# BindsNET/bindsnet

Hardware: AMD Instinct MI355X
Metric: simulated timesteps/sec (whole node), DiehlAndCook2015 784->400 batch32 (higher is better)
Workload: dtype f32

## Files before the change

### bindsnet_amd/csrc/snn_dc2015_async.hip

```cpp
#include <limits.h>
#include <stdlib.h>
#include "snn_dc2015.hpp"
#include "snn_dc2015_tile.hpp"

namespace {

constexpr int ACW = 4;
constexpr int ANT = 512;
constexpr int kCrossRing = 4;
constexpr int kWinRing = 8;
constexpr int kWinGr = 11;
constexpr int kArbRing = 32;
constexpr unsigned kAPoll = 400000u;
constexpr unsigned kAbortPay = 0xFFFFFFFEu;

__device__ __forceinline__ uint32_t win_tag(int e) { return (uint32_t)(e + 1) & 1023u; }

__device__ __forceinline__ void report(int *status, int code) {
    if (status) atomicCAS(status, 0, code);
}

__device__ __forceinline__ const DcCtx &cold(const DcCtx &) {
    const __attribute__((address_space(4))) DcCtx *p = (const __attribute__((address_space(4))) DcCtx *)__builtin_amdgcn_kernarg_segment_ptr();
    asm volatile("" : "+s"(p));
// ... 92 lines not shown
        cb = blk;
    };
#pragma unroll
    for (int u = 0; u < 8; ++u) if (u < nL) add(ix[u], wx[u] * 1.0f, wy[u] * 1.0f);
    for (int u = 8; u < nL; ++u) {
        const int ii2 = (int)lx[st + u];
        add(ii2, ws[ii2 * CW + pq] * 1.0f, DUAL ? ws2[ii2 * CW + pq] * 1.0f : 0.f);
    }
    const int GL = (Nin >> 4) >> 4;
    auto combine = [&](float G) __attribute__((always_inline)) -> float {
        const float G1 = __shfl_down(G, 1, 4), G2 = __shfl_down(G, 2, 4), G3 = __shfl_down(G, 3, 4);
        const float Gs[4] = {G, G1, G2, G3};
        float A2 = 0.0f;
#pragma unroll
        for (int k = 0; k < 4; ++k) if (k < GL) A2 = A2 + Gs[k];
        float Gl = 0.0f;
#pragma unroll
        for (int k = 0; k < 4; ++k) if (k == GL) Gl = Gs[k];
        const float res = ((0.0f + Gl) + A2) + 0.0f;
        return 0.0f + res;
    };
    if (DUAL) out2 = combine(c1_ + c0_);
    return combine(a1 + a0);
}

template <int K>
__device__ __forceinline__ float quad_down(float v) {
    constexpr int ctrl = K == 1 ? 0x39 : (K == 2 ? 0x0E : 0x03);
    return __int_as_float(__builtin_amdgcn_mov_dpp(__float_as_int(v), ctrl, 0xF, 0xF, true));
}

__device__ __forceinline__ float4 x_current_f4(const float *ws, const uint32_t *dg, int B, int Nin, int pb, int pL, bool tailcol) {
    constexpr uint32_t GM = (1u << GCB) - 1u;
    const uint16_t *lstX = (const uint16_t *)dg;
    const uint32_t *rowmask = dg + B * (LX / 2) + 40;
    const uint16_t *arows = (const uint16_t *)(rowmask + Nin);
    const uint16_t *lst2 = arows + 4 * ((Nin + 1) / 2);
    const uint32_t *gcnt = (const uint32_t *)(lst2 + B * LX);
    const uint32_t *gqn = gcnt + B;
    float r[4];
    if (tailcol) {
        const uint32_t gc = gcnt[pb];
        const int st = (pL > 0 ? (int)(gc & GM) : 0) + (pL > 1 ? (int)((gc >> GCB) & GM) : 0) + (pL > 2 ? (int)((gc >> (2 * GCB)) & GM) : 0);
        const int nL = (int)((gc >> (GCB * pL)) & GM);
        const uint16_t *l2 = lst2 + pb * LX;
        const int n4 = Nin >> 2, nfull = n4 >> 4;
        int ix[8]; float4 wx[8];
#pragma unroll
        for (int u = 0; u < 8; ++u) ix[u] = min((int)l2[min(st + u, LX - 1)], Nin - 1);
#pragma unroll
        for (int u = 0; u < 8; ++u) wx[u] = *(const float4 *)(ws + ix[u] * 4);
        float a0[4] = {0.f, 0.f, 0.f, 0.f}, a1[4] = {0.f, 0.f, 0.f, 0.f}, a2[4] = {0.f, 0.f, 0.f, 0.f};
        int cb = -1;
        auto add = [&](int pos, const float4 &w) __attribute__((always_inline)) {
            int blk = pos >> 4;
            blk = blk < nfull ? blk : nfull;
            const bool nb = blk != cb, ng = (blk >> 4) != (cb >> 4);
            const float t[4] = {w.x * 1.0f, w.y * 1.0f, w.z * 1.0f, w.w * 1.0f};
#pragma unroll
            for (int q = 0; q < 4; ++q) {
                const float s1 = a1[q] + a0[q];
                a1[q] = nb ? s1 : a1[q];
                a0[q] = nb ? 0.f : a0[q];
                const float s2 = a2[q] + a1[q];
                a2[q] = ng ? s2 : a2[q];
                a1[q] = ng ? 0.f : a1[q];
                a0[q] += t[q];
            }
            cb = blk;
        };
#pragma unroll
        for (int u = 0; u < 8; ++u) if (u < nL) add(ix[u] >> 2, wx[u]);
        for (int u = 8; u < nL; ++u) {
            const int i = (int)l2[st + u];
            add(i >> 2, *(const float4 *)(ws + i * 4));
        }
        const bool closeb = cb != nfull, closeg = closeb && (nfull >> 4) != (cb >> 4);
        float v[4];
#pragma unroll
        for (int q = 0; q < 4; ++q) {
            float b0 = a0[q], b1 = a1[q], b2 = a2[q];
            if (closeb) { b1 += b0; b0 = 0.f; if (closeg) { b2 += b1; b1 = 0.f; } }
            v[q] = ((b0 + b1) + b2) + 0.0f;
        }
        if (pL == 0) {
            const int s4 = (int)(gc & GM) + (int)((gc >> GCB) & GM) + (int)((gc >> (2 * GCB)) & GM) + (int)((gc >> (3 * GCB)) & GM);
            const int n5 = (int)((gc >> (4 * GCB)) & GM);
            for (int u = 0; u < n5; ++u) {
                const int i = (int)l2[s4 + u];
                const float4 w = *(const float4 *)(ws + i * 4);
                v[0] += w.x * 1.0f; v[1] += w.y * 1.0f; v[2] += w.z * 1.0f; v[3] += w.w * 1.0f;
            }
        }
#pragma unroll
        for (int q = 0; q < 4; ++q) {
            const float v1 = __shfl_down(v[q], 1, 4), v2 = __shfl_down(v[q], 2, 4), v3 = __shfl_down(v[q], 3, 4);
            r[q] = 0.0f + (((v[q] + v1) + v2) + v3);
        }
        return make_float4(r[0], r[1], r[2], r[3]);
    }
    const uint32_t gq = gqn[pb];
    const int st = (pL > 0 ? (int)(gq & GM) : 0) + (pL > 1 ? (int)((gq >> GCB) & GM) : 0) + (pL > 2 ? (int)((gq >> (2 * GCB)) & GM) : 0);
    const int nL = (int)((gq >> (GCB * pL)) & GM);
    const uint16_t *lx = lstX + pb * LX;
    int ix[8]; float4 wx[8];
    const int last = st + max(nL, 1) - 1;
#pragma unroll
    for (int u = 0; u < 8; ++u) ix[u] = (int)lx[min(st + u, last)];
#pragma unroll
    for (int u = 0; u < 8; ++u) wx[u] = *(const float4 *)(ws + ix[u] * 4);
    float a0[4] = {0.f, 0.f, 0.f, 0.f}, a1[4] = {0.f, 0.f, 0.f, 0.f};
    int cb = -1;
    const int nfull = Nin >> 4;
    auto add = [&](int pos, const float4 &w, float live) __attribute__((always_inline)) {
        int blk = pos >> 4;
        blk = blk < nfull ? blk : nfull;
        const float same = blk == cb ? 1.f : 0.f, diff = 1.f - same;
        const float t[4] = {w.x * live, w.y * live, w.z * live, w.w * live};
#pragma unroll
        for (int q = 0; q < 4; ++q) {
            a1[q] = __builtin_fmaf(a0[q], diff, a1[q]);
            a0[q] = __builtin_fmaf(a0[q], same, t[q]);
        }
        cb = blk;
    };
#pragma unroll
    for (int u = 0; u < 8; ++u) add(ix[u], wx[u], u < nL ? 1.0f : 0.0f);
    for (int u = 8; u < nL; ++u) {
        const int i2 = (int)lx[st + u];
        add(i2, *(const float4 *)(ws + i2 * 4), 1.0f);
    }
    const int GL = (Nin >> 4) >> 4;
#pragma unroll
    for (int q = 0; q < 4; ++q) {
        const float G = a1[q] + a0[q];
        const float G1 = quad_down<1>(G), G2 = quad_down<2>(G), G3 = quad_down<3>(G);
        const float Gs[4] = {G, G1, G2, G3};
        float A2 = 0.0f;
#pragma unroll
        for (int k = 0; k < 4; ++k) if (k < GL) A2 = A2 + Gs[k];
        float Gl = 0.0f;
#pragma unroll
        for (int k = 0; k < 4; ++k) if (k == GL) Gl = Gs[k];
        const float res = ((0.0f + Gl) + A2) + 0.0f;
        r[q] = 0.0f + res;
    }
    return make_float4(r[0], r[1], r[2], r[3]);
}

__device__ __forceinline__ void scan_entry(const DcCtx &c, int *w0, int *cnt0, int tid) {
    const int B = c.B, N = c.N;
    if (tid < 2 * MAXB) { w0[tid] = -1; cnt0[tid] = 0; }
    __syncthreads();
    for (int k = tid; k < B * N; k += ANT) {
        if (c.sE[k]) { const int b = k / N; atomicAdd(&cnt0[b], 1); w0[b] = k - b * N; }
        if (c.sI[k]) { const int b = k / N; atomicAdd(&cnt0[MAXB + b], 1); w0[MAXB + b] = k - b * N; }
    }
    __syncthreads();
}

constexpr int kWinPollSleep = 1;
struct WinPre { unsigned long long g0; bool have; };
__device__ __forceinline__ WinPre win_prefetch(const DcCtx &c, int e, int myb) {
    WinPre p; p.g0 = granule_load(c.wing + (size_t)(e & (kWinRing - 1)) * kWinGr + myb / 3); p.have = true;
    return p;
}
__device__ __forceinline__ int sample_winner(const DcCtx &c, const int *w0, int e, int myb, bool &bad, WinPre pre = WinPre{0ull, false}) {
    if (e < 0) return w0[(e == -1 ? 0 : MAXB) + myb];
    const unsigned long long *gr = c.wing + (size_t)(e & (kWinRing - 1)) * kWinGr + myb / 3;
    const uint32_t tag = win_tag(e);
    unsigned long long x0 = pre.have ? pre.g0 : granule_load(gr);
    for (unsigned spins = 0; __any((uint32_t)(x0 >> 54) != tag); ++spins) {
        if (spins > kAPoll) { bad = true; report(cold(c).status, SNN_ERR_TIMEOUT); return -1; }
        __builtin_amdgcn_s_sleep(kWinPollSleep);
        x0 = granule_load(gr);
    }
    if (__any((int)((x0 >> 48) & 63u) == 63)) { bad = true; return -1; }
    const uint32_t w = (uint32_t)(x0 >> (16 * (myb % 3))) & 0xFFFFu;
    return w == 0xFFFFu ? -1 : (int)(w & 0x7FFu);
}

#define AMARKW(k, th) do { if constexpr (TIMING) { if (c.dbg && g == c.dbg_wg && tid == (th)) c.dbg[(size_t)t * 24 + (k)] = (long long)wall_clock64(); } } while (0)
#define AMARK(k) do { if constexpr (TIMING) { if (wave == 0 && c.dbg_wg >= 0) mk[k] = (long long)wall_clock64(); } } while (0)
#define AMARK2(k) do { if constexpr (TIMING) { if (wave == 2 && c.dbg_wg >= 0) mk[k] = (long long)wall_clock64(); } } while (0)
#define AMARK2_FLUSH() do { if constexpr (TIMING) { if (c.dbg && g == c.dbg_wg && tid == 128 && t >= 1) { _Pragma("unroll") for (int k_ = 19; k_ < 24; ++k_) c.dbg[(size_t)(t - 1) * 24 + k_] = mk[k_]; } } } while (0)
#define AMARK_FLUSH() do { if constexpr (TIMING) { if (c.dbg && g == c.dbg_wg && tid == 0) { _Pragma("unroll") for (int k_ = 0; k_ < 19; ++k_) { \
        const bool early_ = k_ == 0 || k_ == 9 || k_ == 10 || k_ == 7 || k_ == 11 || k_ == 18; \
        if (k_ != 3 && k_ != 17 && (early_ || t >= 1)) c.dbg[(size_t)(early_ ? t : t - 1) * 24 + k_] = mk[k_]; } } } } while (0)

__device__ __forceinline__ float vgpr(float x) { float r; asm volatile("v_mov_b32 %0, %1" : "=v"(r) : "s"(x)); return r; }
__device__ __forceinline__ snn_lif_params vgpr_params(snn_lif_params p) {
    p.decay = vgpr(p.decay); p.rest = vgpr(p.rest); p.reset = vgpr(p.reset); p.thresh = vgpr(p.thresh); p.refrac = vgpr(p.refrac);
    p.dt = vgpr(p.dt); p.lbound = vgpr(p.lbound); p.trace_decay = vgpr(p.trace_decay); p.trace_scale = vgpr(p.trace_scale);
    return p;
}
struct PPar { float nu0, nu1, dt, wmin, wmax; int use_dt, has_min, has_max; };

__device__ __forceinline__ float4 postpre_row_nowin(const PPar &c, float4 w4, uint32_t m, const float *xnu0) {
    float w[4] = {w4.x, w4.y, w4.z, w4.w};
    if (c.nu0 != 0.f) {
        float a0[4] = {0.f, 0.f, 0.f, 0.f}, a1[4] = {0.f, 0.f, 0.f, 0.f};
        int cblk = 0;
        while (m) {
            const int b = __ffs(m) - 1; m &= m - 1;
            const float4 xn = *(const float4 *)(xnu0 + b * 4);
            const float xv[4] = {xn.x, xn.y, xn.z, xn.w};
            const float same = (b >> 4) == cblk ? 1.f : 0.f, diff = 1.f - same;
            cblk = b >> 4;
#pragma unroll
            for (int q = 0; q < 4; ++q) {
                a1[q] = __builtin_fmaf(a0[q], diff, a1[q]);
                a0[q] = __builtin_fmaf(a0[q], same, 1.0f * xv[q]);
            }
        }
#pragma unroll
        for (int q = 0; q < 4; ++q) {
            float uu = ((a0[q] + a1[q]) + 0.f) + 0.0f;
            if (c.use_dt) uu = uu * c.dt;
            w[q] = w[q] - uu;
        }
    }
    if (c.nu1 != 0.f) {
#pragma unroll
        for (int q = 0; q < 4; ++q) {
            float uu = 0.f;
            if (c.use_dt) uu = uu * c.dt;
            w[q] = w[q] + uu;
        }
    }
#pragma unroll
    for (int q = 0; q < 4; ++q) {
        if (c.has_min && w[q] < c.wmin) w[q] = c.wmin;
        if (c.has_max && w[q] > c.wmax) w[q] = c.wmax;
    }
    return make_float4(w[0], w[1], w[2], w[3]);
}

__device__ __forceinline__ float postpre_elem(const PPar &c, int B, int Nin, const float *xnu0, float w, int i, int q, uint32_t m, uint32_t cm,
                                              int bst, float xw, const float *xs, bool have_x, float xval) {
    constexpr int CW = ACW;
    if (c.nu0 != 0.f) {
        float uu = 0.f;
        if (m) {
            CascadeT acc; acc.init(false);
            while (m) {
                const int b = __ffs(m) - 1; m &= m - 1;
                acc.add(b, 1.0f * (b == bst ? xw : xnu0[b * CW + q]), B);
            }
            uu = acc.finish(B);
        }
        if (c.use_dt) uu = uu * c.dt;
        w = w - uu;
    }
    if (c.nu1 != 0.f) {
        float uu = 0.f;
        if (cm) {
            CascadeT acc; acc.init(false);
            while (cm) {
                const int b = __ffs(cm) - 1; cm &= cm - 1;
                acc.add(b, (have_x ? xval : xs[b * Nin + i]) * (1.0f * c.nu1), B);
            }
            uu = acc.finish(B);
        }
        if (c.use_dt) uu = uu * c.dt;
        w = w + uu;
    }
    if (c.has_min && w < c.wmin) w = c.wmin;
    if (c.has_max && w > c.wmax) w = c.wmax;
    return w;
}

constexpr int kXChunk = 256;
__device__ __forceinline__ int x_chunks(const DcCtx &c) { return c.x_traces ? (c.B * c.Nin + kXChunk - 1) / kXChunk : 0; }

__device__ __forceinline__ void async_producer(const DcCtx &c, unsigned char *smem, int p) {
    const int T = c.T, tid = threadIdx.x;
    for (int e = p; e <= T; e += c.NP) {
        const int flags = dc_prep_entry<ANT>(c, smem, e, c.dig + (size_t)e * c.DW);
        if (tid == 0) {
            if (flags & 5) atomicOr(c.tbad, 1);
            __hip_atomic_store(&c.dready[e], (flags & 5) ? 2 : 1, __ATOMIC_RELEASE, __HIP_MEMORY_SCOPE_AGENT);
            __hip_atomic_fetch_add(&c.dready[T + 1], 1, __ATOMIC_RELEASE, __HIP_MEMORY_SCOPE_AGENT);
        }
    }
    const int n = c.B * c.Nin, nch = x_chunks(c);
    for (int ch = p; ch < nch; ch += c.NP) {
        const int k = ch * kXChunk + tid;
        if (tid < kXChunk && k < n) { if (c.x_additive) xtrace_body<true>(c, n, k); else xtrace_body<false>(c, n, k); }
        __syncthreads();
        if (tid == 0) __hip_atomic_fetch_add(&c.dready[T + 2], 1, __ATOMIC_RELEASE, __HIP_MEMORY_SCOPE_AGENT);
    }
    if (c.rasX) {
        const size_t n16 = ((size_t)T * c.B * c.Nin) >> 4;
        const uint4 *src = (const uint4 *)c.in;
        uint4 *dst = (uint4 *)c.rasX;
        for (size_t k = (size_t)p * ANT + tid; k < n16; k += (size_t)c.NP * ANT) dst[k] = src[k];
    }
}

__device__ __forceinline__ int need_entry(const DcCtx &c, int e, bool &all) {
    const int T = c.T;
    int r;
    if (__hip_atomic_load(&c.dready[T + 1], __ATOMIC_RELAXED, __HIP_MEMORY_SCOPE_AGENT) == T + 1) {
        all = true;
        r = 0;
    } else {
        for (unsigned spins = 0;; ++spins) {
            r = __hip_atomic_load(&c.dready[e], __ATOMIC_RELAXED, __HIP_MEMORY_SCOPE_AGENT);
            if (r) break;
            if (spins > kAPoll) return -1;
            __builtin_amdgcn_s_sleep(4);
        }
    }
    __builtin_amdgcn_fence(__ATOMIC_ACQUIRE, "agent");
    if (all) r = __hip_atomic_load(c.tbad, __ATOMIC_RELAXED, __HIP_MEMORY_SCOPE_AGENT) != 0 ? 2 : 1;
    return r;
}
__device__ __forceinline__ int need_xtr(const DcCtx &c, bool &all) {
    const int nch = x_chunks(c);
    for (unsigned spins = 0;; ++spins) {
        if (__hip_atomic_load(&c.dready[c.T + 2], __ATOMIC_RELAXED, __HIP_MEMORY_SCOPE_AGENT) == nch) break;
        if (spins > kAPoll) return -1;
        __builtin_amdgcn_s_sleep(4);
    }
    __builtin_amdgcn_fence(__ATOMIC_ACQUIRE, "agent");
    all = true;
    return 1;
}

template <bool TIMING, bool FT>
__device__ __forceinline__ void async_compute(const DcCtx &c, unsigned char *smem) {
    constexpr int CW = ACW, TT = AT, NT = ANT, NTW = TT / 64, SPW = 64 / CW, SPG = 16 / CW, NBC = NT - TT, TI0 = NT - TT;
    const int B = FT ? MAXB : c.B, Nin = c.Nin, N = c.N, T = c.T;
    int *ctl = (int *)(smem + OC_CTL);
    float *xnu0 = (float *)(smem + OC_XNU0);
    float *xnu0s = (float *)(smem + OC_XNU0S);
    float *curX = (float *)(smem + OC_CURX);
    float *curXwin = (float *)(smem + OC_CURXW);
    int *spfin = (int *)(smem + OC_SPFIN);
    int *thc = (int *)(smem + OC_THC);
    uint32_t *colmask = (uint32_t *)(smem + OC_COLM);
    uint32_t *colx = (uint32_t *)(smem + OC_COLX);
    uint32_t *colres = (uint32_t *)(smem + OC_COLRES);
    float *xwinv = (float *)(smem + OC_XWINV);
    int *xcnt = (int *)(smem + OC_XCNT);
    int *w0 = (int *)(smem + OC_W0), *cnt0 = (int *)(smem + OC_C0);
    float *wtile = (float *)(smem + OC_WT);
    float *wieT = wtile + (size_t)Nin * CW;
    float *weiT = wieT + (size_t)N * CW;
    const int DGS = (c.DGW + 63) & ~63;
    uint32_t *dgbuf = (uint32_t *)(weiT + (size_t)N * CW);
    float *wbak = (float *)(dgbuf + 2 * DGS);
    float *wwin = wbak + (size_t)Nin * CW;

    const int tid = threadIdx.x, lane = tid & 63, wave = tid >> 6;
    const int g = (int)blockIdx.x, c0 = g * CW;
    const bool is_ai = tid >= TI0;
    const int ptile = is_ai ? tid - TI0 : tid;
    const int jj = ptile % CW, bl = ptile / CW, j = c0 + jj;
    const bool colv = FT ? true : j < N, tailcol = c0 >= (N / 32) * 32;
    const bool mine = FT ? tid < TT : (tid < TT && bl < B && colv);
    const bool mine_i = FT ? is_ai : (is_ai && bl < B && colv);
    const unsigned kst = (unsigned)(bl * N + j);
    const int NGS = c.G * NTW;
    const snn_lif_params pE = vgpr_params(c.pE.lif), pI = vgpr_params(c.pI);
    const float theta_plus = vgpr(c.pE.theta_plus), theta_decay = vgpr(c.pE.theta_decay);
    const PPar pp = {vgpr(c.nu0), vgpr(c.nu1), vgpr(c.dt), vgpr(c.wmin), vgpr(c.wmax), c.use_dt, c.has_min, c.has_max};
    const bool e_learning = c.pE.learning != 0;

    if (tid < 32) ctl[tid] = 0;
    if (tid < 2 * CW) { thc[tid] = 0; colx[tid] = 0; colmask[tid] = 0; colres[tid & 3] = 0; xwinv[tid & 3] = 0.f; }
    scan_entry(c, w0, cnt0, tid);
    bool offdiag = false, multi0 = false;
    for (int k = tid; k < Nin * CW; k += NT) {
        const int i = k / CW, q = k % CW;
        wtile[k] = (c0 + q < N) ? c.Wxe[i * N + c0 + q] : 0.f;
        wbak[k] = 0.f; wwin[k] = 0.f;
    }
    for (int k = tid; k < N * CW; k += NT) {
        const int i = k / CW, q = k % CW;
        wieT[k] = (c0 + q < N) ? c.Wie[i * N + c0 + q] : 0.f;
        const float we = (c0 + q < N) ? c.Wei[i * N + c0 + q] : 0.f;
        weiT[k] = we;
        offdiag = offdiag || (i != c0 + q && we != 0.f);
    }
    if (tid < 2 * MAXB) multi0 = cnt0[tid] > 1;
    if (offdiag || multi0) ctl[0] = 1;
    const int nchunk = c.DGW >> 2;
    uint4 dg0 = make_uint4(0, 0, 0, 0), dg1 = dg0, dg2 = dg0;
#define DIGEST_LOAD(e) do { const uint4 *src_ = (const uint4 *)(c.dig + (size_t)(e) * c.DW); dg0 = src_[min(tid, nchunk - 1)]; \
                            dg1 = src_[min(tid + NT, nchunk - 1)]; dg2 = src_[min(tid + 2 * NT, nchunk - 1)]; } while (0)
#define DIGEST_STORE(e) do { uint4 *dst_ = (uint4 *)(dgbuf + ((e) & 1) * DGS); if (tid < nchunk) dst_[tid] = dg0; \
                             if (tid + NT < nchunk) dst_[tid + NT] = dg1; if (tid + 2 * NT < nchunk) dst_[tid + 2 * NT] = dg2; } while (0)
    int pend = 0;
    int dig01 = 1;
    if (c.NP != 0) {
        bool dig_all = false;
        const int r0 = need_entry(c, 0, dig_all), r1 = (T >= 1 && !dig_all) ? need_entry(c, 1, dig_all) : 1;
        dig01 = r0 != 1 ? r0 : r1;
        if (dig01 != 1) { ctl[0] = 1; if (tid == 0) report(c.status, dig01 < 0 ? SNN_ERR_TIMEOUT : SNN_ERR_RETRY); }
        const int p0 = (dig_all ? 0 : 1) | (c.x_traces ? 2 : 0);
        asm volatile("v_mov_b32 %0, %1" : "=v"(pend) : "s"(p0));
    }
#define PENDING(bit) (__builtin_amdgcn_readfirstlane(pend) & (bit))
    if (dig01 >= 0) DIGEST_LOAD(0);
    DIGEST_STORE(0);
    if (T >= 1) { if (dig01 >= 0) DIGEST_LOAD(1); DIGEST_STORE(1); }
    uint4 dg3 = make_uint4(0, 0, 0, 0);
#define DIGEST_LOAD_E(e) do { const uint4 *src_ = (const uint4 *)(c.dig + (size_t)(e) * c.DW); const int d_ = tid - TT; dg0 = src_[min(d_, nchunk - 1)]; \
                              dg1 = src_[min(d_ + NBC, nchunk - 1)]; dg2 = src_[min(d_ + 2 * NBC, nchunk - 1)]; dg3 = src_[min(d_ + 3 * NBC, nchunk - 1)]; } while (0)
#define DIGEST_STORE_E(e) do { uint4 *dst_ = (uint4 *)(dgbuf + ((e) & 1) * DGS); const int d_ = tid - TT; if (d_ < nchunk) dst_[d_] = dg0; \
                               if (d_ + NBC < nchunk) dst_[d_ + NBC] = dg1; if (d_ + 2 * NBC < nchunk) dst_[d_ + 2 * NBC] = dg2; \
                               if (d_ + 3 * NBC < nchunk) dst_[d_ + 3 * NBC] = dg3; } while (0)
    float r_v = 0.f, r_r = 0.f, r_th = 0.f, x_cur = 0.f, x_before = 0.f;
    bool last_s = false;
    if (mine) {
        r_v = c.vE[kst]; r_r = c.rE[kst]; r_th = c.theta[j];
        x_cur = pE.traces ? c.xE[kst] : 0.f;
        last_s = c.sE[kst] != 0;
    }
    if (mine_i) {
        r_v = c.vI[kst]; r_r = c.rI[kst];
        x_cur = pI.traces ? c.xI[kst] : 0.f;
        last_s = c.sI[kst] != 0;
    }
    if (tid < TT) {
        float xn = 0.f;
        if (bl < B && colv && pE.traces) xn = trace_next(x_cur, 0, pE.trace_decay, pE.trace_scale, pE.traces_additive);
        xnu0[tid] = xn * pp.nu0; xnu0[TT + tid] = 0.f; xnu0s[tid] = 0.f;
        curX[tid] = 0.f; curX[TT + tid] = 0.f; curXwin[tid] = 0.f;
        spfin[tid] = (mine && last_s) ? 1 : 0;
    }
    asm volatile("s_waitcnt vmcnt(0)" ::: "memory");
    __syncthreads();
    bool bad = ctl[0] != 0;
    if (bad && tid == 0) report(c.status, SNN_ERR_RETRY);
    for (int qt = tid; qt < B * CW * 4; qt += NT) {
        const int pb = qt / (CW * 4), pq = (qt >> 2) % CW, pL = qt & 3;
        float unused = 0.f;
        const float v = x_current4<false>(wtile, wtile, unused, dgbuf, B, Nin, pb, pq, pL, tailcol);
        if (pL == 0 && c0 + pq < N) curX[pb * CW + pq] = v;
    }
    lds_barrier();
    bool sp_prev = false;
    bool crossed_prev = false;
    unsigned long long prevE = 0ull;
    int published = 0;
    WinPre pre_w = WinPre{0ull, false};
    const bool learn_pp = c.learning && c.rule == SNN_RULE_POSTPRE;

    if constexpr (TIMING) {
        if (c.dbg && tid == 0) {
            c.dbg[(size_t)24 * (T + 1) + ((size_t)T * 256 + g) * 4 + 2] = (long long)(__builtin_amdgcn_s_getreg((31 << 11) | 20) & 0xF);
            c.dbg[(size_t)24 * (T + 1) + ((size_t)T * 256 + g) * 4 + 3] = (long long)(__builtin_amdgcn_s_getreg((31 << 11) | 4) & 0xFFFFFF);
        }
    }
    long long mk[24] = {0, 0, 0, 0, 0, 0, 0, 0, 0, 0, 0, 0, 0, 0, 0, 0, 0, 0, 0, 0, 0, 0, 0, 0};
    (void)mk;
    bool prev_anyx = true;
    auto step_loop = [&](auto role_c) __attribute__((always_inline)) {
    constexpr int ROLE = decltype(role_c)::value;
    constexpr bool R_TILE = ROLE == 0, R_F4 = ROLE == 1, R_W4 = ROLE == 2, R_AI = ROLE == 3, R_NT = ROLE != 0;
    (void)R_W4; (void)R_AI; (void)R_F4;
    for (int t = 0; t <= T; ++t) {
        const bool phaseB = t < T;
        const int par = t & 1;
        const uint32_t *dgn = dgbuf + (par ^ 1) * DGS;
        const int *meta = (const int *)(dgn + B * (LX / 2));
        const uint32_t *rowmask = dgn + B * (LX / 2) + 40;
        const uint16_t *arows = (const uint16_t *)(rowmask + Nin);
        const bool do_stdp = phaseB && learn_pp;
        const bool full = t == 0;
        AMARK(0);
        AMARK2_FLUSH();
        if constexpr (TIMING) { if (c.dbg && tid == 0 && c.dbg_wg >= 0) c.dbg[(size_t)24 * (T + 1) + ((size_t)t * 256 + g) * 4 + 0] = (long long)wall_clock64(); }
        if (t + 2 <= T && R_NT) {
            if (PENDING(1)) {
                bool all = false;
                const int r = need_entry(cold(c), t + 2, all);
                if (r != 1) { ctl[0] = 1; report(cold(c).status, r < 0 ? SNN_ERR_TIMEOUT : SNN_ERR_RETRY); }
                if (all) pend &= ~1;
            }
            DIGEST_LOAD_E(t + 2);
        }
        float cx_plain = 0.f;
        int thc_prev = 0;
        if (R_TILE) { cx_plain = curX[par * TT + tid]; thc_prev = thc[(par ^ 1) * CW + jj]; }
        if (ctl[0]) { bad = true; break; }
        AMARK(9);
        uint32_t wonm = 0;
        if (learn_pp && prev_anyx) {
#pragma unroll
            for (int q = 0; q < CW; ++q) wonm |= (__builtin_amdgcn_readfirstlane((int)colmask[par * CW + q]) != 0 ? 1u : 0u) << q;
        }
        AMARK(10);
        if (!phaseB) {
            if (wonm)
                for (int i = tid; i < Nin; i += NT) {
                    float4 v = *(const float4 *)(wtile + i * 4);
                    const float4 ww = *(const float4 *)(wwin + i * 4);
                    if (wonm & 1u) v.x = ww.x;
                    if (wonm & 2u) v.y = ww.y;
                    if (wonm & 4u) v.z = ww.z;
                    if (wonm & 8u) v.w = ww.w;
                    *(float4 *)(wtile + i * 4) = v;
                }
            break;
        }
        if (R_TILE) {
// ... 162 lines not shown
                }
                lds_barrier();
#pragma unroll
                for (int q = 0; q < CW; ++q) if (__popc(xq[q]) > 1) cmq[q] = (uint32_t)__builtin_amdgcn_readfirstlane((int)colres[q]);
                if (R_TILE) {
                    float v = xn0[tid];
                    const uint32_t xj = jj == 0 ? xq[0] : (jj == 1 ? xq[1] : (jj == 2 ? xq[2] : xq[3]));
                    const uint32_t cj = jj == 0 ? cmq[0] : (jj == 1 ? cmq[1] : (jj == 2 ? cmq[2] : cmq[3]));
                    if (bl < B && colv && __popc(xj) > 1 && ((cj >> bl) & 1u) && pE.traces)
                        v = trace_next(x_before, 1, pE.trace_decay, pE.trace_scale, pE.traces_additive) * pp.nu0;
                    xnu0s[tid] = v;
                }
                lds_barrier();
            }
            if (!f4w)
                for (int k = R_TILE ? tid : tid - 128; k < nact; k += NT - 128) {
                    const int i = full ? k : (int)arows[k];
#pragma unroll
                    for (int q = 0; q < CW; ++q) if (cmq[q] && c0 + q < N) won_elem(i, q);
                }
            AMARK2(20);
            lds_barrier();
        }
        AMARK(15);
        if (crossed_wg && R_W4) {
            const int ptid = tid - TT - 128, pb = ptid >> 2, pL = ptid & 3;
            const float4 v = x_current_f4(wwin, dgn, B, Nin, min(pb, B - 1), pL, tailcol);
            if (pL == 0 && pb < B) {
                if (cmq[0] && c0 + 0 < N) curXwin[pb * CW + 0] = v.x;
                if (cmq[1] && c0 + 1 < N) curXwin[pb * CW + 1] = v.y;
                if (cmq[2] && c0 + 2 < N) curXwin[pb * CW + 2] = v.z;
                if (cmq[3] && c0 + 3 < N) curXwin[pb * CW + 3] = v.w;
            }
        }
        AMARK(5);
        AMARK2(21);

        if (crossed_wg && R_NT && !full) {
            for (int i = tid - TT; i < Nin; i += NBC) {
                if (rowmask[i] != 0) continue;
#pragma unroll
                for (int q = 0; q < CW; ++q) if (cmq[q] && c0 + q < N) won_elem(i, q);
            }
        }
        AMARK(6);
        AMARK2(22);
        if (R_TILE) {
            sp_prev = false;
            if (prevE != 0ull && !bad) {
                int *xc = xcnt + wave * MAXB;

                if (lane < MAXB) xc[lane] = 0;
                {
                    constexpr int PG = 8;
                    const unsigned long long *sums = cold(c).exs + (size_t)(t & (kCrossRing - 1)) * NGS;
                    unsigned long long xs[PG];
                    uint32_t need = 0;
#pragma unroll
                    for (int u = 0; u < PG; ++u) { xs[u] = 0ull; if (lane + 64 * u < NGS) need |= 1u << u; }
                    for (unsigned spins = 0;; ++spins) {
#pragma unroll
                        for (int u = 0; u < PG; ++u) if ((need >> u) & 1u) xs[u] = granule_load(sums + lane + 64 * u);
#pragma unroll
                        for (int u = 0; u < PG; ++u) if (((need >> u) & 1u) && (uint32_t)(xs[u] >> 32) == (uint32_t)(t + 1)) need &= ~(1u << u);
                        if (!__any(need != 0u)) break;
                        if (spins > kAPoll) { bad = true; report(cold(c).status, SNN_ERR_TIMEOUT); break; }
                    }
                    bool ab = false;
#pragma unroll
                    for (int u = 0; u < PG; ++u) {
                        const int gi = lane + 64 * u;
                        if (bad || gi >= NGS) continue;
                        const uint32_t pay = (uint32_t)xs[u];
                        if (!pay) continue;
                        if (pay == kAbortPay) { ab = true; continue; }
                        const int w = gi % NTW;
                        if ((pay & 0xFFu) == 0xFFu) {
                            for (int bs = 0; bs < SPW; ++bs) if (w * SPW + bs < B) atomicAdd(&xc[w * SPW + bs], 2);
                        } else {
                            const int ne = (int)(pay >> 30);
                            for (int e2 = 0; e2 < ne; ++e2) {
                                const int bsm = w * SPW + (int)((pay >> (8 * e2)) & 0x3Fu) / CW;
                                if (bsm < B) atomicAdd(&xc[bsm], 1);
                            }
                        }
                    }
                    if (__any(ab)) bad = true;
                }
                asm volatile("s_waitcnt lgkmcnt(0)" ::: "memory");
                const int mycnt = (crossed_prev && bl < B) ? xc[bl] : 0;
                int jw = (crossed_prev && mycnt == 1) ? j : -1;
                if (!bad && __any(crossed_prev && mycnt > 1)) {
                    const int ja = sample_winner(c, w0, t, min(bl, B - 1), bad);
                    if (mycnt > 1) jw = ja;
                }
                const bool sp = !bad && crossed_prev && jw == j && bl < B && colv;
                if (sp) {
                    if (pE.traces) {
                        x_cur = trace_next(x_before, 1, pE.trace_decay, pE.trace_scale, pE.traces_additive);
                        if (t + 1 < T) xnu0[(par ^ 1) * TT + tid] = trace_next(x_cur, 0, pE.trace_decay, pE.trace_scale, pE.traces_additive) * pp.nu0;
                    }
                    atomicOr(&colmask[(par ^ 1) * CW + jj], 1u << bl);
                    last_s = true; sp_prev = true;
                }
            }
            spfin[tid] = sp_prev ? 1 : 0;
            if (bad) ctl[0] = 1;
        }
        AMARK(1);

        AMARK(16);
        AMARK2(23);
        lds_barrier();
        AMARK(2);
    }
    };
    if (wave < NTW) step_loop(std::integral_constant<int, 0>{});
    else if (wave < NTW + 2) step_loop(std::integral_constant<int, 1>{});
    else if (wave < NTW + 4) step_loop(std::integral_constant<int, 2>{});
    else step_loop(std::integral_constant<int, 3>{});
    if (PENDING(2) && !bad) {
        bool all = false;
        if (need_xtr(cold(c), all) != 1) { bad = true; report(cold(c).status, SNN_ERR_TIMEOUT); }
    }
    if (wave < NTW && lane == 0) {
        const int pstep = (bad && published <= T - 1) ? published : T;
        granule_store(c.exs + (size_t)(pstep & (kCrossRing - 1)) * NGS + g * NTW + wave, ((unsigned long long)(uint32_t)(pstep + 1) << 32) | (bad ? kAbortPay : 0u));
    }
    asm volatile("s_waitcnt vmcnt(0)" ::: "memory");
    if (wave == 0 && !bad) {
        bool b2 = false;
        (void)sample_winner(c, w0, T, 0, b2);
        if (!b2 && lane == 0) ctl[1] = 1;
    }
    __syncthreads();
    if (ctl[0] != 0 || ctl[1] == 0) return;
    if (c.x_traces) {
        const float *src = c.xtr + (size_t)T * B * Nin;
        for (int k = g * NT + tid; k < B * Nin; k += c.G * NT) c.xX[1][k] = src[k];
    }
    if (mine) {
        float th = r_th;
        if (e_learning) th = th + theta_plus * (float)thc[((T - 1) & 1) * CW + jj];
        c.vE[kst] = r_v; c.rE[kst] = r_r;
        if (bl == 0) c.theta[j] = th;
        if (pE.traces) c.xE[kst] = x_cur;
        c.sE[kst] = last_s;
    }
    if (mine_i) {
        c.vI[kst] = r_v; c.rI[kst] = r_r;
        if (pI.traces) c.xI[kst] = x_cur;
        c.sI[kst] = last_s;
    }
    if (c.has_norm) {
        float *bsum = (float *)dgbuf;
        float *sc = xnu0;
        const int nfull = Nin >> 4;
        __syncthreads();
        if (!tailcol) {
            for (int item = tid; item < nfull * CW; item += NT) {
                const int blk = item / CW, q = item % CW;
                float a0 = 0.f;
#pragma unroll
                for (int k = 0; k < 16; ++k) { const float w = wtile[(blk * 16 + k) * CW + q]; a0 += c.norm_abs ? fabsf(w) : w; }
                bsum[item] = a0;
            }
            __syncthreads();
            if (tid < CW) {
                float a1 = 0.f, a2 = 0.f, a3 = 0.f;
                for (int blk = 0; blk < nfull; ++blk) {
                    a1 += bsum[blk * CW + tid];
                    const int m = blk + 1;
                    if ((m & 15) == 0) { a2 += a1; a1 = 0.f; if ((m & 255) == 0) { a3 += a2; a2 = 0.f; } }
                }
                float a0 = 0.f;
                for (int i = nfull * 16; i < Nin; ++i) { const float w = wtile[i * CW + tid]; a0 += c.norm_abs ? fabsf(w) : w; }
                float cs = ((a0 + a1) + a2) + a3;
                if (cs == 0.f) cs = 1.0f;
                sc[tid] = (1.0f / cs) * c.norm;
            }
        } else {
            __syncthreads();
            if (tid < CW * 4) {
                const int q = tid >> 2, s4 = tid & 3, n4 = Nin >> 2, nf4 = n4 >> 4;
                Cascade cc; cc.init();
                for (int p_ = 0; p_ < n4; ++p_) { const float w = wtile[(4 * p_ + s4) * CW + q]; cc.add(p_, c.norm_abs ? fabsf(w) : w, nf4); }
                float lsum = cc.finish(nf4);
                if (s4 == 0)
                    for (int i = n4 * 4; i < Nin; ++i) { const float w = wtile[i * CW + q]; lsum += c.norm_abs ? fabsf(w) : w; }
                const float l1 = __shfl_down(lsum, 1, 4), l2 = __shfl_down(lsum, 2, 4), l3 = __shfl_down(lsum, 3, 4);
                float cs = ((lsum + l1) + l2) + l3;
                if (cs == 0.f) cs = 1.0f;
                if (s4 == 0) sc[q] = (1.0f / cs) * c.norm;
            }
        }
        __syncthreads();
        for (int k = tid; k < Nin * CW; k += NT) {
            const int i = k / CW, q = k % CW;
            if (c0 + q < N) c.Wxe[i * N + c0 + q] = wtile[k] * sc[q];
        }
    } else if (c.learning && c.rule == SNN_RULE_POSTPRE) {
        for (int k = tid; k < Nin * CW; k += NT) {
            const int i = k / CW, q = k % CW;
            if (c0 + q < N) c.Wxe[i * N + c0 + q] = wtile[k];
        }
    }
}


__device__ __forceinline__ int arb_sample(const DcCtx &c, const uint32_t *mt, int tb, int off, int r, const uint32_t *crsrow,
                                          unsigned long long *key, int lane) {
    constexpr int RMK = kArbRing - 1;
    const int N = c.N, NW = c.NW;
    const uint32_t bits = lane < NW ? crsrow[lane] : 0u;
    unsigned long long k1 = ~0ull, k2 = ~0ull;
    for (uint32_t bb = bits; bb; bb &= bb - 1) {
        const int jx = lane * 32 + __ffs(bb) - 1;
        const int w0 = off + 2 * (r * N + jx), w1 = w0 + 1;
        const int m0 = w0 / 624, m1 = w1 / 624;
        const uint32_t hi = mt_temper(mt[((tb + m0) & RMK) * 624 + w0 - 624 * m0]);
        const uint32_t lo = mt_temper(mt[((tb + m1) & RMK) * 624 + w1 - 624 * m1]);
        const unsigned long long m = (((unsigned long long)hi << 32) | lo) & ((1ull << 53) - 1ull);
        const unsigned long long kk = (m << 10) | (unsigned long long)jx;
        if (kk < k1) { k2 = k1; k1 = kk; } else if (kk < k2) k2 = kk;
    }
    if (lane == 0) *key = ~0ull;
    if (bits) atomicMin(key, k1);
    asm volatile("s_waitcnt lgkmcnt(0)" ::: "memory");
    const unsigned long long kmin = *(volatile unsigned long long *)key;
    const unsigned long long mmin = kmin >> 10, zone = mmin + (mmin >> c.zone_shift) + 1ull;
    const bool close = (k1 != ~0ull && k1 != kmin && (k1 >> 10) <= zone) || (k2 != ~0ull && (k2 >> 10) <= zone);
    int win = (int)(kmin & 1023ull);
    if (__any(close)) {
        if (lane == 0) *key = 0ull;
        for (uint32_t bb = bits; bb; bb &= bb - 1) {
            const int jx = lane * 32 + __ffs(bb) - 1;
            const int w0 = off + 2 * (r * N + jx), w1 = w0 + 1;
            const int m0 = w0 / 624, m1 = w1 / 624;
            const float q = exp1_from_words(mt_temper(mt[((tb + m0) & RMK) * 624 + w0 - 624 * m0]),
                                            mt_temper(mt[((tb + m1) & RMK) * 624 + w1 - 624 * m1]));
            const float val = 1.0f / q;
            atomicMax(key, ((unsigned long long)__float_as_uint(val) << 32) | (uint32_t)(0xFFFFFFFFu - (uint32_t)jx));
        }
        asm volatile("s_waitcnt lgkmcnt(0)" ::: "memory");
        win = (int)(0xFFFFFFFFu - (uint32_t)(*(volatile unsigned long long *)key & 0xFFFFFFFFull));
    }
    return win;
}

template <bool TIMING>
__device__ __forceinline__ void async_arbiter(const DcCtx &c, unsigned char *smem) {
    constexpr int CW = ACW, NTW = AT / 64, SPW = 64 / CW, SPG = 16 / CW, RB = kArbRing, RMK = RB - 1;
    const int B = c.B, N = c.N, NW = c.NW, T = c.T, G = c.G;
    int *ctl = (int *)(smem + OA_CTL);
    int *cntc = (int *)(smem + OA_CNT), *colc = (int *)(smem + OA_COL), *winlist = (int *)(smem + OA_WL);
    unsigned long long *keys = (unsigned long long *)(smem + OA_KEY);
    uint32_t *crs = (uint32_t *)(smem + OA_CRS);
    const int BW = B * NW, BWp = (BW + 3) & ~3;
    uint32_t *mt = crs + BWp;
    const int tid = threadIdx.x, lane = tid & 63, wave = tid >> 6;
    const int KB = c.KB, NG = G * KB, NGS = G * NTW;

    if (tid < 32) { ctl[tid] = 0; cntc[tid] = 0; colc[tid] = 0; }
    for (int k = tid; k < BW; k += ANT) crs[k] = 0;
    for (int k = tid; k < 624; k += ANT) mt[k] = c.rng[0]->mt[k];
    __syncthreads();
    if (wave == 1) {
        for (int k = 1;; ++k) {
            bool stop = false;
            for (;;) {
                if (k - __hip_atomic_load(&ctl[1], __ATOMIC_RELAXED, __HIP_MEMORY_SCOPE_WORKGROUP) < RB) break;
                if (__hip_atomic_load(&ctl[2], __ATOMIC_RELAXED, __HIP_MEMORY_SCOPE_WORKGROUP)) { stop = true; break; }
                __builtin_amdgcn_s_sleep(2);
            }
            if (stop || __hip_atomic_load(&ctl[2], __ATOMIC_RELAXED, __HIP_MEMORY_SCOPE_WORKGROUP)) break;
            asm volatile("" ::: "memory");
            mt_twist_block_wave(mt + ((k - 1) & RMK) * 624, mt + (k & RMK) * 624, lane);
            asm volatile("s_waitcnt lgkmcnt(0)" ::: "memory");
            if (lane == 0) __hip_atomic_store(&ctl[0], k, __ATOMIC_RELAXED, __HIP_MEMORY_SCOPE_WORKGROUP);
        }
    } else if (wave == 0) {
        int pos = __builtin_amdgcn_readfirstlane(c.rng[0]->pos);
        int tb = 0;
        long long consumed;
        {
            const long long c0_ = c.rng[0]->consumed;
            consumed = ((long long)__builtin_amdgcn_readfirstlane((int)(c0_ >> 32)) << 32) | (unsigned)__builtin_amdgcn_readfirstlane((int)c0_);
        }
        bool failed = false;
        auto wait_block = [&](int need) __attribute__((always_inline)) -> bool {
            for (unsigned spins = 0; __hip_atomic_load(&ctl[0], __ATOMIC_RELAXED, __HIP_MEMORY_SCOPE_WORKGROUP) < need; ++spins) {
                if (spins > 40000000u) return false;
                __builtin_amdgcn_s_sleep(1);
            }
            asm volatile("" ::: "memory");
            return true;
        };
        auto publish_abort = [&](int e0) __attribute__((always_inline)) {
            if (lane < 3 * kWinGr) {
                const int de = lane / kWinGr, k = lane - de * kWinGr;
                granule_store(c.wing + (size_t)((e0 + de) & (kWinRing - 1)) * kWinGr + k,
                              ((unsigned long long)win_tag(e0 + de) << 54) | (63ull << 48) | 0xFFFFFFFFFFFFull);
            }
        };
        auto raster_wait = [&](int e0, int rp) __attribute__((always_inline)) -> bool {
            bool late = false;
            if (c.NRW > 0 && e0 >= kWinRing - 2 && lane < c.NRW) {
                for (unsigned spins = 0; rp < e0 - (kWinRing - 2) + 1; ++spins) {
                    if (spins > kAPoll) { late = true; break; }
                    __builtin_amdgcn_s_sleep(1);
                    rp = __hip_atomic_load(&c.rprog[lane], __ATOMIC_RELAXED, __HIP_MEMORY_SCOPE_AGENT);
                }
            }
            return __any(late);
        };
        int e = 0;
        for (; e < T && !failed; ++e) {
            const int slot = e & (kCrossRing - 1);
            const unsigned long long *sums = c.exs + (size_t)slot * NGS;
            const unsigned long long *exr = c.ex + (size_t)slot * NG;
            bool abortseen = false;

            int rp = INT_MAX;
            if (c.NRW > 0 && lane < c.NRW) rp = __hip_atomic_load(&c.rprog[lane], __ATOMIC_RELAXED, __HIP_MEMORY_SCOPE_AGENT);
            constexpr int PG = 8;
            unsigned long long xs[PG];
            uint32_t need = 0;
#pragma unroll
            for (int u = 0; u < PG; ++u) { xs[u] = 0ull; if (lane + 64 * u < NGS) need |= 1u << u; }
            for (unsigned spins = 0;; ++spins) {
#pragma unroll
                for (int u = 0; u < PG; ++u) if ((need >> u) & 1u) xs[u] = granule_load(sums + lane + 64 * u);
#pragma unroll
                for (int u = 0; u < PG; ++u) if (((need >> u) & 1u) && (uint32_t)(xs[u] >> 32) == (uint32_t)(e + 1)) need &= ~(1u << u);
                if (!__any(need != 0u)) break;
                if (spins > kAPoll) { failed = true; break; }
            }
            auto event = [&](int bsm, int jx) __attribute__((always_inline)) {
                if (bsm >= B || jx >= N) return;
                atomicOr((unsigned int *)&crs[bsm * NW + (jx >> 5)], 1u << (jx & 31));
                atomicAdd(&cntc[bsm], 1);
                colc[bsm] = jx;
            };
#pragma unroll
            for (int u = 0; u < PG; ++u) {
                const int gi = lane + 64 * u;
                if (failed || gi >= NGS) continue;
                const uint32_t pay = (uint32_t)xs[u];
                if (!pay) continue;
                if (pay == kAbortPay) { abortseen = true; continue; }
                const int gsrc = gi / NTW, w = gi - gsrc * NTW;
                if ((pay & 0xFFu) == 0xFFu) {
                    for (int q = 0; q < SPW / SPG; ++q) {
                        const int k = w * (SPW / SPG) + q;
// ... 4 lines not shown
                            if ((uint32_t)(d >> 32) == (uint32_t)(e + 1)) break;
                            if (sp2 > kAPoll) { failed = true; break; }
                            __builtin_amdgcn_s_sleep(1);
                        }
                        if (failed) break;
                        uint32_t be = (uint32_t)d & 0xFFFFu;
                        while (be) { const int p_ = __ffs(be) - 1; be &= be - 1; event(k * SPG + p_ / CW, gsrc * CW + p_ % CW); }
                    }
                } else {
                    const int ne = (int)(pay >> 30);
                    for (int e2 = 0; e2 < ne; ++e2) {
                        const uint32_t ev = (pay >> (8 * e2)) & 0xFFu;
                        const int p_ = (int)(ev & 0x3Fu);
                        event(w * SPW + p_ / CW, gsrc * CW + p_ % CW);
                    }
                }
            }
            failed = __any(failed);
            abortseen = __any(abortseen);
            if constexpr (TIMING) { if (c.dbg && lane == 0) c.dbg[(size_t)24 * (T + 1) + ((size_t)e * 256 + 255) * 4 + 0] = (long long)wall_clock64(); }
            if (failed) { if (lane == 0) report(c.status, SNN_ERR_TIMEOUT); }
            if (failed || abortseen) {
                (void)raster_wait(e, rp);
                publish_abort(e);
                failed = true;
                break;
            }
            asm volatile("s_waitcnt lgkmcnt(0)" ::: "memory");
            const int myc = lane < B ? cntc[lane] : 0;
            int mywin = (lane < B && myc == 1) ? colc[lane] : -1;
            const uint32_t anym = (uint32_t)__ballot(myc > 0);
            const uint32_t multim = (uint32_t)__ballot(myc > 1);
            const int arb_rows = __popc(anym);
            for (uint32_t rem = multim; rem; rem &= rem - 1) {
                const int bsm = __ffs(rem) - 1;
                const int r = __popc(anym & ((1u << bsm) - 1u));
                const int first = tb + (pos + 2 * r * N) / 624, lastb = tb + (pos + 2 * (r + 1) * N - 1) / 624;
                if (lane == 0) __hip_atomic_store(&ctl[1], first, __ATOMIC_RELAXED, __HIP_MEMORY_SCOPE_WORKGROUP);
                if (!wait_block(lastb)) { failed = true; break; }
                const int wcol = arb_sample(c, mt, tb, pos, r, crs + bsm * NW, &keys[bsm], lane);
                if (lane == bsm) mywin = wcol;
            }
            if (failed) {
                if (lane == 0) report(c.status, SNN_ERR_TIMEOUT);
                publish_abort(e);
                break;
            }
            if (lane < 32) winlist[lane] = (lane < B && myc > 0) ? ((lane << 11) | (mywin & 0x7FF)) : 0xFFFF;
            asm volatile("s_waitcnt lgkmcnt(0)" ::: "memory");
            if (raster_wait(e, rp)) {
                if (lane == 0) report(c.status, SNN_ERR_TIMEOUT);
                publish_abort(e);
                failed = true;
                break;
            }
            if (lane < kWinGr) {
                unsigned long long pl = 0;
#pragma unroll
                for (int u = 0; u < 3; ++u) {
                    const int idx = 3 * lane + u;
                    const unsigned long long wv = idx < 32 ? (unsigned long long)(uint32_t)winlist[idx] : 0xFFFFull;
                    pl |= wv << (16 * u);
                }
                granule_store(c.wing + (size_t)(e & (kWinRing - 1)) * kWinGr + lane,
                              ((unsigned long long)win_tag(e) << 54) | ((unsigned long long)arb_rows << 48) | pl);
            }
            if constexpr (TIMING) { if (c.dbg && lane == 0) { c.dbg[(size_t)24 * (T + 1) + ((size_t)e * 256 + 255) * 4 + 1] = (long long)wall_clock64(); c.dbg[(size_t)24 * (T + 1) + ((size_t)e * 256 + 255) * 4 + 2] = arb_rows + 100 * __popc(multim); } }
            if (arb_rows) {
                const int endw = pos + 2 * arb_rows * N;
                const int adv = (endw - 1) / 624;
                tb += adv; pos = endw - 624 * adv;
                consumed += (long long)arb_rows * N;
                if (lane == 0) __hip_atomic_store(&ctl[1], tb, __ATOMIC_RELAXED, __HIP_MEMORY_SCOPE_WORKGROUP);
                for (int k = lane; k < BW; k += 64) crs[k] = 0;
                if (lane < 32) cntc[lane] = 0;
            }
        }
        if (!failed && e == T) {
            {
                const unsigned long long *sums = c.exs + (size_t)(T & (kCrossRing - 1)) * NGS;
                bool ab = false, to = false;
                for (int gi = lane; gi < NGS; gi += 64) {
                    unsigned long long x = granule_load(sums + gi);
                    for (unsigned spins = 0; (uint32_t)(x >> 32) != (uint32_t)(T + 1); ++spins) {
                        if (spins > kAPoll) { to = true; break; }
                        __builtin_amdgcn_s_sleep(1);
                        x = granule_load(sums + gi);
                    }
                    if (to) break;
                    if ((uint32_t)x == kAbortPay) ab = true;
                }
                if (__any(to)) { if (lane == 0) report(c.status, SNN_ERR_TIMEOUT); failed = true; }
                else if (__any(ab)) failed = true;
                if (failed) { (void)raster_wait(T, 0); publish_abort(T); }
            }
        }
        if (!failed && e == T) {
            bool late = false;
            if (c.NRW > 0 && lane < c.NRW) {
                for (unsigned spins = 0; __hip_atomic_load(&c.rprog[lane], __ATOMIC_RELAXED, __HIP_MEMORY_SCOPE_AGENT) < T; ++spins) {
                    if (spins > kAPoll) { late = true; break; }
                    __builtin_amdgcn_s_sleep(1);
                }
            }
            if (__any(late) || !wait_block(tb)) {
                if (lane == 0) report(c.status, SNN_ERR_TIMEOUT);
                publish_abort(T);
            } else {
                if (lane == 0)
                    granule_store(c.wing + (size_t)(T & (kWinRing - 1)) * kWinGr, ((unsigned long long)win_tag(T) << 54) | 0xFFFFFFFFFFFFull);
                snn_rng_state *wr = c.rng[0];
                for (int k = lane; k < 624; k += 64) wr->mt[k] = mt[(tb & RMK) * 624 + k];
                if (lane == 0) { wr->pos = pos; wr->consumed = consumed; }
            }
        }
        if (lane == 0) __hip_atomic_store(&ctl[2], 1, __ATOMIC_RELAXED, __HIP_MEMORY_SCOPE_WORKGROUP);
    }
}

__device__ __forceinline__ void async_raster(const DcCtx &c, unsigned char *smem, int rid) {
    const int B = c.B, N = c.N, T = c.T;
    int *w0 = (int *)smem, *cnt0 = w0 + 2 * MAXB;
    int *wcur = cnt0 + 2 * MAXB;
    int *flag = wcur + 2 * MAXB;
    const int tid = threadIdx.x, lane = tid & 63, wave = tid >> 6, NWV = ANT / 64;
    scan_entry(c, w0, cnt0, tid);
    if (tid < MAXB) { wcur[MAXB + tid] = w0[tid]; wcur[tid] = -1; }
    if (tid == 0) flag[0] = 0;
    __syncthreads();
    for (int e = 0; e < T; ++e) {
        const int par = e & 1;
        if (wave == 0) {
            bool bad = false;
            const int wv = sample_winner(c, w0, e, min(lane, B - 1), bad);
            if (lane < MAXB) wcur[par * MAXB + lane] = lane < B ? wv : -1;
            if (bad && lane == 0) flag[0] = 1;
        }
        lds_barrier();
        if (flag[0]) break;
        for (int r = rid + c.NRW * wave; r < 2 * B; r += c.NRW * NWV) {
            const int b = r < B ? r : r - B;
            uint8_t *ras = r < B ? c.rasE : c.rasI;
            const int jw = r < B ? wcur[par * MAXB + b] : wcur[(par ^ 1) * MAXB + b];
            if (ras) { uint8_t *row = ras + ((size_t)e * B + b) * N; for (int jx = lane; jx < N; jx += 64) row[jx] = (uint8_t)(jx == jw); }
        }
        lds_barrier();
        if (tid == 0) __hip_atomic_store(&c.rprog[rid], e + 1, __ATOMIC_RELAXED, __HIP_MEMORY_SCOPE_AGENT);
    }
}

template <bool TIMING, bool FT>
__global__ __launch_bounds__(ANT) void k_dc2015_async(const DcCtx c) {
    extern __shared__ __attribute__((aligned(16))) unsigned char smem[];
    const int blk = (int)blockIdx.x;
    if (blk == c.stall_wg) return;
    if (c.NP == 0 && *c.tbad != 0) {
        if (blk == 0 && threadIdx.x == 0) report(c.status, SNN_ERR_RETRY);
        return;
    }
    if (blk < c.G) async_compute<TIMING, FT>(c, smem);
    else if (blk == c.G) async_arbiter<TIMING>(c, smem);
    else if (blk < c.G + 1 + c.NRW) async_raster(c, smem, blk - c.G - 1);
    else async_producer(c, smem, blk - c.G - 1 - c.NRW);
}

}

size_t snn_dc2015_async_lds(int B, int Nin, int N) {
    const size_t a = async_compute_lds(B, Nin, N), b = async_arbiter_lds(B, N), p = dc_prep_lds_bytes(B, Nin, ANT);
    return a > b ? (a > p ? a : p) : (b > p ? b : p);
}

static bool async_attr_once() {
    static int state = 0;
    if (!state) state = (snn_check(hipFuncSetAttribute((const void *)k_dc2015_async<false, false>, hipFuncAttributeMaxDynamicSharedMemorySize, 150 * 1024)) ||
                         snn_check(hipFuncSetAttribute((const void *)k_dc2015_async<false, true>, hipFuncAttributeMaxDynamicSharedMemorySize, 150 * 1024)) ||
                         snn_check(hipFuncSetAttribute((const void *)k_dc2015_async<true, false>, hipFuncAttributeMaxDynamicSharedMemorySize, 150 * 1024))) ? -1 : 1;
    return state == 1;
}

int snn_dc2015_async_capacity(size_t lds) {
    if (!async_attr_once()) return 0;
    int dev = 0;
    if (hipGetDevice(&dev) != hipSuccess) return 0;
    struct Known { int dev; size_t lds; int cap; };
    static thread_local Known known[4] = {{-1, 0, 0}, {-1, 0, 0}, {-1, 0, 0}, {-1, 0, 0}};
    static thread_local int next = 0;
    const char *fake = getenv("SNN_DC_FAKE_CUS");
    const int fake_cus = fake ? atoi(fake) : 0;
    if (!fake_cus) for (const Known &k : known) if (k.dev == dev && k.lds == lds) return k.cap;
    int cus = 0, coop = 0, per_cu = 0;
    if (hipDeviceGetAttribute(&cus, hipDeviceAttributeMultiprocessorCount, dev) != hipSuccess) return 0;
    if (hipDeviceGetAttribute(&coop, hipDeviceAttributeCooperativeLaunch, dev) != hipSuccess) coop = 0;
    if (hipOccupancyMaxActiveBlocksPerMultiprocessor(&per_cu, (const void *)k_dc2015_async<false, false>, ANT, lds) != hipSuccess) { (void)hipGetLastError(); return 0; }
    if (fake_cus) cus = fake_cus;
    const int cap = coop ? cus * per_cu : 0;
    if (!fake_cus) { known[next] = Known{dev, lds, cap}; next = (next + 1) & 3; }
    return cap;
}

int snn_dc2015_async_launch(const DcCtx &c, size_t lds, hipStream_t st, bool ordinary) {
    if (!async_attr_once()) return SNN_ERR_LAUNCH;
    static const bool coop_env = !(getenv("SNN_DC_COOP") && atoi(getenv("SNN_DC_COOP")) == 0);
    const bool coop = coop_env && !ordinary;
    DcCtx arg = c;
    void *args[1] = {(void *)&arg};
    const unsigned grid = (unsigned)(c.G + 1 + c.NRW + c.NP);
    static const bool ft_env = !(getenv("SNN_DC_FULLTILE") && atoi(getenv("SNN_DC_FULLTILE")) == 0);
    const bool ft = ft_env && c.B == MAXB && c.N % ACW == 0;
    const void *fn = c.dbg ? (const void *)k_dc2015_async<true, false>
                           : (ft ? (const void *)k_dc2015_async<false, true> : (const void *)k_dc2015_async<false, false>);
    if (!coop) return snn_check(hipLaunchKernel(fn, dim3(grid), dim3(ANT), args, lds, st));
    const hipError_t e = hipLaunchCooperativeKernel(fn, dim3(grid), dim3(ANT), args, (unsigned)lds, st);
    if (e == hipErrorCooperativeLaunchTooLarge) { (void)hipGetLastError(); return SNN_ERR_UNSUPPORTED; }
    return snn_check(e);
}
```

Baseline: 294,000.

## Vectorize spike scan and weight writeback, remap producer blocks to launch first

```diff
diff --git a/bindsnet_amd/csrc/snn_dc2015_async.hip b/bindsnet_amd/csrc/snn_dc2015_async.hip
--- a/bindsnet_amd/csrc/snn_dc2015_async.hip
+++ b/bindsnet_amd/csrc/snn_dc2015_async.hip
@@ -268,9 +268,27 @@
     const int B = c.B, N = c.N;
     if (tid < 2 * MAXB) { w0[tid] = -1; cnt0[tid] = 0; }
     __syncthreads();
-    for (int k = tid; k < B * N; k += ANT) {
-        if (c.sE[k]) { const int b = k / N; atomicAdd(&cnt0[b], 1); w0[b] = k - b * N; }
-        if (c.sI[k]) { const int b = k / N; atomicAdd(&cnt0[MAXB + b], 1); w0[MAXB + b] = k - b * N; }
+    const int n = B * N;
+    auto hit = [&](int base, int k) __attribute__((always_inline)) { const int b = k / N; atomicAdd(&cnt0[base + b], 1); w0[base + b] = k - b * N; };
+    auto piece = [&](int base, int k16, const uint4 &v) __attribute__((always_inline)) {
+        if (!(v.x | v.y | v.z | v.w)) return;
+        const uint32_t w[4] = {v.x, v.y, v.z, v.w};
+#pragma unroll
+        for (int u = 0; u < 4; ++u)
+            for (uint32_t m = nz4(w[u]); m; m &= m - 1) hit(base, k16 * 16 + u * 4 + __ffs(m) - 1);
+    };
+    const bool al16 = (((uintptr_t)c.sE | (uintptr_t)c.sI) & 15) == 0;
+    const int n16 = al16 ? n >> 4 : 0;
+    const uint4 *e16 = (const uint4 *)c.sE, *i16 = (const uint4 *)c.sI;
+    for (int k16 = tid; k16 < n16; k16 += 2 * ANT) {
+        const int k2 = k16 + ANT, k2c = min(k2, n16 - 1);
+        const uint4 ve0 = e16[k16], ve1 = e16[k2c], vi0 = i16[k16], vi1 = i16[k2c];
+        piece(0, k16, ve0); piece(MAXB, k16, vi0);
+        if (k2 < n16) { piece(0, k2, ve1); piece(MAXB, k2, vi1); }
+    }
+    for (int k = n16 * 16 + tid; k < n; k += ANT) {
+        if (c.sE[k]) hit(0, k);
+        if (c.sI[k]) hit(MAXB, k);
     }
     __syncthreads();
 }
@@ -445,7 +463,7 @@
 }
 
 template <bool TIMING, bool FT>
-__device__ __forceinline__ void async_compute(const DcCtx &c, unsigned char *smem) {
+__device__ __forceinline__ void async_compute(const DcCtx &c, unsigned char *smem, const int g) {
     constexpr int CW = ACW, TT = AT, NT = ANT, NTW = TT / 64, SPW = 64 / CW, SPG = 16 / CW, NBC = NT - TT, TI0 = NT - TT;
     const int B = FT ? MAXB : c.B, Nin = c.Nin, N = c.N, T = c.T;
     int *ctl = (int *)(smem + OC_CTL);
@@ -470,7 +488,7 @@
     float *wwin = wbak + (size_t)Nin * CW;
 
     const int tid = threadIdx.x, lane = tid & 63, wave = tid >> 6;
-    const int g = (int)blockIdx.x, c0 = g * CW;
+    const int c0 = g * CW;
     const bool is_ai = tid >= TI0;
     const int ptile = is_ai ? tid - TI0 : tid;
     const int jj = ptile % CW, bl = ptile / CW, j = c0 + jj;
@@ -939,11 +957,12 @@
         if (pI.traces) c.xI[kst] = x_cur;
         c.sI[kst] = last_s;
     }
+    const bool rows4_out = (FT || (N & 3) == 0) && (((uintptr_t)cold(c).Wxe & 15) == 0);
     if (c.has_norm) {
         float *bsum = (float *)dgbuf;
         float *sc = xnu0;
         const int nfull = Nin >> 4;
-        __syncthreads();
+        lds_barrier();
         if (!tailcol) {
             for (int item = tid; item < nfull * CW; item += NT) {
                 const int blk = item / CW, q = item % CW;
@@ -952,13 +971,20 @@
                 for (int k = 0; k < 16; ++k) { const float w = wtile[(blk * 16 + k) * CW + q]; a0 += c.norm_abs ? fabsf(w) : w; }
                 bsum[item] = a0;
             }
-            __syncthreads();
+            lds_barrier();
             if (tid < CW) {
                 float a1 = 0.f, a2 = 0.f, a3 = 0.f;
-                for (int blk = 0; blk < nfull; ++blk) {
-                    a1 += bsum[blk * CW + tid];
-                    const int m = blk + 1;
-                    if ((m & 15) == 0) { a2 += a1; a1 = 0.f; if ((m & 255) == 0) { a3 += a2; a2 = 0.f; } }
+                for (int b0 = 0; b0 < nfull; b0 += 16) {
+                    float bs[16];
+#pragma unroll
+                    for (int u = 0; u < 16; ++u) bs[u] = bsum[min(b0 + u, nfull - 1) * CW + tid];
+#pragma unroll
+                    for (int u = 0; u < 16; ++u)
+                        if (b0 + u < nfull) {
+                            a1 += bs[u];
+                            const int m = b0 + u + 1;
+                            if ((m & 15) == 0) { a2 += a1; a1 = 0.f; if ((m & 255) == 0) { a3 += a2; a2 = 0.f; } }
+                        }
                 }
                 float a0 = 0.f;
                 for (int i = nfull * 16; i < Nin; ++i) { const float w = wtile[i * CW + tid]; a0 += c.norm_abs ? fabsf(w) : w; }
@@ -981,12 +1007,22 @@
                 if (s4 == 0) sc[q] = (1.0f / cs) * c.norm;
             }
         }
-        __syncthreads();
+        lds_barrier();
+        if (rows4_out) {
+            const float4 s4 = *(const float4 *)sc;
+            for (int i = tid; i < Nin; i += NT) {
+                const float4 w = *(const float4 *)(wtile + i * CW);
+                *(float4 *)(c.Wxe + i * N + c0) = make_float4(w.x * s4.x, w.y * s4.y, w.z * s4.z, w.w * s4.w);
+            }
+        } else
         for (int k = tid; k < Nin * CW; k += NT) {
             const int i = k / CW, q = k % CW;
             if (c0 + q < N) c.Wxe[i * N + c0 + q] = wtile[k] * sc[q];
         }
     } else if (c.learning && c.rule == SNN_RULE_POSTPRE) {
+        if (rows4_out) {
+            for (int i = tid; i < Nin; i += NT) *(float4 *)(c.Wxe + i * N + c0) = *(const float4 *)(wtile + i * CW);
+        } else
         for (int k = tid; k < Nin * CW; k += NT) {
             const int i = k / CW, q = k % CW;
             if (c0 + q < N) c.Wxe[i * N + c0 + q] = wtile[k];
@@ -1297,13 +1333,17 @@
 template <bool TIMING, bool FT>
 __global__ __launch_bounds__(ANT) void k_dc2015_async(const DcCtx c) {
     extern __shared__ __attribute__((aligned(16))) unsigned char smem[];
-    const int blk = (int)blockIdx.x;
+    int blk = (int)blockIdx.x;
+    if (c.NP >= 8) {
+        const int first = c.G + 1 + c.NRW;
+        if (blk < 8) blk += first; else if (blk < first + 8) blk -= 8;
+    }
     if (blk == c.stall_wg) return;
     if (c.NP == 0 && *c.tbad != 0) {
         if (blk == 0 && threadIdx.x == 0) report(c.status, SNN_ERR_RETRY);
         return;
     }
-    if (blk < c.G) async_compute<TIMING, FT>(c, smem);
+    if (blk < c.G) async_compute<TIMING, FT>(c, smem, blk);
     else if (blk == c.G) async_arbiter<TIMING>(c, smem);
     else if (blk < c.G + 1 + c.NRW) async_raster(c, smem, blk - c.G - 1);
     else async_producer(c, smem, blk - c.G - 1 - c.NRW);
```

Measured after the change: 289,600. 0.985x the previous value.
